# GabrielGao0310/SVT-av1_pro-anchor-v2.1.0-

Hardware: AMD Instinct MI355X
Metric: CDEF+restoration+SAD Mpixels/s on 4K10b (higher is better)
Workload: dtype u16

## Files before the change

svt-av1_pro-anchor-v2.1.0-_amd/csrc/dlf.hip:

```cpp
#include <algorithm>
#include <cstdlib>
#include <cstring>
#include <vector>

#include "svtgpu_internal.h"

#ifndef DLF_EXP
#define DLF_EXP 0
#endif

namespace {

constexpr int kNumBsize = 22;
__constant__ uint8_t c_tx_lw[3][kNumBsize] = {
    {2, 2, 3, 3, 3, 4, 4, 4, 5, 5, 5, 6, 6, 6, 6, 6, 2, 4, 3, 5, 4, 6},
    {2, 2, 3, 2, 3, 3, 3, 4, 4, 4, 5, 5, 5, 6, 6, 6, 2, 3, 3, 4, 4, 5},
    {2, 2, 3, 3, 2, 2, 2, 3, 3, 3, 4, 4, 4, 6, 6, 6, 2, 2, 3, 3, 4, 4}};
__constant__ uint8_t c_tx_lh[3][kNumBsize] = {
    {2, 3, 2, 3, 4, 3, 4, 5, 4, 5, 6, 5, 6, 6, 6, 6, 4, 2, 5, 3, 6, 4},
    {2, 3, 2, 2, 3, 3, 3, 4, 4, 4, 5, 5, 5, 6, 6, 6, 3, 2, 4, 3, 5, 4},
    {2, 3, 2, 3, 2, 2, 2, 3, 3, 3, 4, 4, 4, 6, 6, 6, 2, 2, 3, 3, 4, 4}};
__constant__ uint8_t c_uvtx_lw[kNumBsize] = {2, 2, 2, 2, 2, 3, 3, 3, 4, 4, 4, 5, 5, 5, 5, 5, 2, 3, 2, 4, 3, 5};
__constant__ uint8_t c_uvtx_lh[kNumBsize] = {2, 2, 2, 2, 3, 2, 3, 4, 3, 4, 5, 4, 5, 5, 5, 5, 3, 2, 4, 2, 5, 3};
__constant__ uint8_t c_bs_lw[kNumBsize]   = {2, 2, 3, 3, 3, 4, 4, 4, 5, 5, 5, 6, 6, 6, 7, 7, 2, 4, 3, 5, 4, 6};
__constant__ uint8_t c_bs_lh[kNumBsize]   = {2, 3, 2, 3, 4, 3, 4, 5, 4, 5, 6, 5, 6, 7, 6, 7, 4, 2, 5, 3, 6, 4};
__constant__ uint8_t c_uvbs_lw[kNumBsize] = {2, 2, 2, 2, 2, 3, 3, 3, 4, 4, 4, 5, 5, 5, 6, 6, 2, 3, 2, 4, 3, 5};
__constant__ uint8_t c_uvbs_lh[kNumBsize] = {2, 2, 2, 2, 3, 2, 3, 4, 3, 4, 5, 4, 5, 6, 5, 6, 3, 2, 4, 2, 5, 3};
__device__ __forceinline__ int mode_lf(int mode) { return mode >= 13 && mode != 15 && mode != 23; }

__device__ __forceinline__ int lf_class(const SvtGpuLfMi &m) {
    return m.segment_id * 16 + m.ref_frame0 * 2 + mode_lf(m.mode);
}

__device__ __forceinline__ int tx_log2(const SvtGpuLfMi &m, int vert, int chroma) {
    const int skipped = m.skip && m.ref_frame0 > 0;
    if (chroma) return vert ? c_uvtx_lw[m.bsize] : c_uvtx_lh[m.bsize];
    const int d = skipped ? 0 : m.tx_depth;
    return vert ? c_tx_lw[d][m.bsize] : c_tx_lh[d][m.bsize];
}

__device__ __forceinline__ SvtGpuLfMi checked_mi(SvtGpuLfMi m, unsigned long long *bad) {
    if (bad && (m.bsize >= kNumBsize || m.tx_depth > 2 || m.ref_frame0 < 0 || m.ref_frame0 > 7 || m.mode > 24 ||
                m.segment_id > 7)) {
        *bad = 1;
        m.bsize = min((int)m.bsize, kNumBsize - 1), m.tx_depth = min((int)m.tx_depth, 2);
        m.ref_frame0 = (int8_t)min(max((int)m.ref_frame0, 0), 7), m.mode = min((int)m.mode, 24);
        m.segment_id = min((int)m.segment_id, 7);
    }
    return m;
}

__global__ void dlf_edge_records_kernel(const SvtGpuLfMi *__restrict__ mi, int mi_cols, int units_w, int units_h,
                                        int chroma, int vert, int crop_w, int crop_h, uint32_t *__restrict__ rec,
                                        unsigned long long *bad) {
    const int ux = blockIdx.x * blockDim.x + threadIdx.x;
    const int uy = blockIdx.y;
    if (ux >= units_w || uy >= units_h) return;
    const int ss     = chroma;
    const int x      = ux * 4, y = uy * 4;
    const int mi_row = ss | ((y << ss) >> 2), mi_col = ss | ((x << ss) >> 2);
    const SvtGpuLfMi m = checked_mi(mi[mi_row * mi_cols + mi_col], bad);
    const int coord    = vert ? x : y;
    uint32_t  r        = 0;
    const int lt       = tx_log2(m, vert, chroma);
    if (coord && !(coord & ((1 << lt) - 1)) && x < crop_w && y < crop_h) {
        const SvtGpuLfMi p = checked_mi(vert ? mi[mi_row * mi_cols + mi_col - (1 << ss)]
                                             : mi[(mi_row - (1 << ss)) * mi_cols + mi_col], bad);
        const int cur_skip = m.skip && m.ref_frame0 > 0;
        const int pv_skip  = p.skip && p.ref_frame0 > 0;
        const int lpb      = chroma ? (vert ? c_uvbs_lw[m.bsize] : c_uvbs_lh[m.bsize])
                                    : (vert ? c_bs_lw[m.bsize] : c_bs_lh[m.bsize]);
        const int pu_edge  = !(coord & ((1 << lpb) - 1));
        if (!pv_skip || !cur_skip || pu_edge) {
            const int mlt = min(lt, tx_log2(p, vert, chroma));
            const int len = mlt == 2 ? 4 : chroma ? 6 : mlt == 3 ? 8 : 14;
            r = (uint32_t)len | ((uint32_t)lf_class(m) << 8) | ((uint32_t)lf_class(p) << 16);
        }
    }
    rec[(size_t)uy * units_w + ux] = r;
}

__device__ __forceinline__ int sclamp(int v, int lo, int hi) { return min(max(v, lo), hi); }

template <int N, int LOG2>
__device__ __forceinline__ void wide_filter(int *F) {
    int out[2 * N];
#pragma unroll
    for (int i = -N; i < N; i++) {
        int t = 0;
#pragma unroll
        for (int j = -N; j <= N; j++) {
            const int p   = min(max(i + j, -(N + 1)), N);
            const int tap = (N == 3 ? j == 0 : (j >= -1 && j <= 1)) ? 2 : 1;
            t += F[p + 7] * tap;
        }
        out[i + N] = (t + (1 << (LOG2 - 1))) >> LOG2;
    }
#pragma unroll
    for (int i = -N; i < N; i++) F[i + 7] = out[i + N];
}

__device__ __forceinline__ void filter_line(int *F, int len, int blimit, int limit, int thresh, int bd) {
    const int sh = bd - 8, one = 1 << sh;
    const int p3 = F[3], p2 = F[4], p1 = F[5], p0 = F[6], q0 = F[7], q1 = F[8], q2 = F[9], q3 = F[10];
    const int lim = limit << sh;
    if (abs(p0 - q0) * 2 + abs(p1 - q1) / 2 > (blimit << sh)) return;
    int m = max(abs(p1 - p0), abs(q1 - q0));
    int flat = 0;
    if (len >= 6) {
        m = max(m, max(abs(p2 - p1), abs(q2 - q1)));
        flat = max(max(abs(p1 - p0), abs(q1 - q0)), max(abs(p2 - p0), abs(q2 - q0)));
    }
    if (len >= 8) {
        m    = max(m, max(abs(p3 - p2), abs(q3 - q2)));
        flat = max(flat, max(abs(p3 - p0), abs(q3 - q0)));
    }
    if (m > lim) return;
    if (len >= 6 && flat <= one) {
        if (len == 14) {
            const int flat2 = max(max(max(abs(F[2] - p0), abs(F[11] - q0)), max(abs(F[1] - p0), abs(F[12] - q0))),
                                  max(abs(F[0] - p0), abs(F[13] - q0)));
            if (flat2 <= one) {
                wide_filter<6, 4>(F);
                return;
            }
        }
        if (len == 6)
            wide_filter<2, 3>(F);
        else
            wide_filter<3, 3>(F);
        return;
    }
    const int off = 0x80 << sh, lo = -(128 << sh), hi = (128 << sh) - 1;
    const bool hev = max(abs(p1 - p0), abs(q1 - q0)) > (thresh << sh);
    const int ps1 = p1 - off, ps0 = p0 - off, qs0 = q0 - off, qs1 = q1 - off;
    int f = hev ? sclamp(ps1 - qs1, lo, hi) : 0;
    f            = sclamp(f + 3 * (qs0 - ps0), lo, hi);
    const int f1 = sclamp(f + 4, lo, hi) >> 3;
    const int f2 = sclamp(f + 3, lo, hi) >> 3;
    F[7]         = sclamp(qs0 - f1, lo, hi) + off;
    F[6]         = sclamp(ps0 + f2, lo, hi) + off;
    if (!hev) {
        const int f3 = (f1 + 1) >> 1;
        F[8]         = sclamp(qs1 - f3, lo, hi) + off;
        F[5]         = sclamp(ps1 + f3, lo, hi) + off;
    }
}

__device__ __forceinline__ int half_taps(int len) { return len == 14 ? 7 : len == 8 ? 4 : len == 6 ? 3 : 2; }

constexpr int TILE  = 64;
constexpr int APRON = 12;
constexpr int LW    = TILE + 2 * APRON;
constexpr int NTHR  = 256;
constexpr int MAX_TRIALS = 2;

constexpr int MAX_JOBS   = 3;

struct DlfPlaneJob {
    int32_t         plane;
    const void     *src;
    void           *dst;
    const void     *ref;
    const uint32_t *rec_v, *rec_h;
    int32_t         src_stride, dst_stride, ref_stride;
    int32_t         units_w;
    int32_t         pw, ph, tiles_x, tiles;
    int32_t         ox, oy, ow, oh;
    int32_t         ntrial;
    uint8_t         lvl[MAX_TRIALS][2][128];
};

struct DlfDevPlan {
    int32_t ntrial[MAX_JOBS];
    int32_t lv[MAX_JOBS][MAX_TRIALS];
    uint8_t lvl[MAX_JOBS][MAX_TRIALS][2][128];
    int32_t done;
};

struct DlfTileArgs {
    DlfPlaneJob job[MAX_JOBS];
    int32_t     njob, bd;
    uint8_t     mblim[64], lim[64], hev[64];
    unsigned long long *sse;
    unsigned int       *arrive;
    unsigned long long *out;
    unsigned long long  seq;
    unsigned long long *wgclk;
    const DlfDevPlan   *plan;
    DlfDevPlan         *next_plan = nullptr;
    int32_t             dyn;
    const uint8_t      *dev_lvl;
};

typedef const __attribute__((address_space(4))) DlfTileArgs KArgs;
typedef const __attribute__((address_space(4))) DlfPlaneJob KJob;
__device__ __forceinline__ KArgs &kargs() { return *(KArgs *)__builtin_amdgcn_kernarg_segment_ptr(); }

struct DlfTileLds {
    uint16_t t[LW * LW];
    uint32_t rv[(LW / 4) * (TILE / 4 + 3)];
    uint32_t rh[(TILE / 4 + 3) * (TILE / 4)];
    unsigned long long red[NTHR / 64];
    uint8_t  s_lvl[2][128];
    uint32_t s_thr[64];
    uint16_t s_list[(LW / 4) * (TILE / 4 + 3)];
    int      s_cnt[8];
};

__device__ __forceinline__ int list_edges(const uint32_t *rec, int n, const uint8_t *lvl, uint16_t *list, int *s_cnt) {
    const int tid = threadIdx.x, lane = tid & 63;
    auto bucket = [&](int ri) {
        const uint32_t r   = rec[ri];
        const int      len = r & 15;
        if (!len || (!lvl[(r >> 8) & 127] && !lvl[(r >> 16) & 127])) return -1;
        return len == 4 ? 0 : len == 6 ? 1 : len == 8 ? 2 : 3;
    };
    if (tid < 8) s_cnt[tid] = 0;
    __syncthreads();
    for (int i0 = 0; i0 < n; i0 += NTHR) {
        const int b = i0 + tid < n ? bucket(i0 + tid) : -1;
#pragma unroll
        for (int g = 0; g < 4; g++) {
            const unsigned long long m = __ballot(b == g);
            if (m && lane == __ffsll((long long)m) - 1) atomicAdd(&s_cnt[g], (int)__popcll(m));
        }
    }
    __syncthreads();
    if (tid == 0) {
        int o = 0;
        for (int g = 0; g < 4; g++) {
            const int c = s_cnt[g];
            s_cnt[4 + g] = o, s_cnt[g] = o, o += c;
        }
    }
    __syncthreads();
    for (int i0 = 0; i0 < n; i0 += NTHR) {
        const int b = i0 + tid < n ? bucket(i0 + tid) : -1;
#pragma unroll
        for (int g = 0; g < 4; g++) {
            const unsigned long long m = __ballot(b == g);
            if (!m) continue;
            const int leader = __ffsll((long long)m) - 1;
            int       base   = 0;
            if (lane == leader) base = atomicAdd(&s_cnt[g], (int)__popcll(m));
            base = __shfl(base, leader);
            if (b == g) list[base + __popcll(m & ((1ull << lane) - 1))] = (uint16_t)(i0 + tid);
        }
    }
    __syncthreads();
    return s_cnt[3];
}

template <typename T, bool TRIAL>
__device__ __forceinline__ void dlf_tile_item(KArgs &a, int bi, int nbi, DlfTileLds &L) {
    uint16_t           *t = L.t;
    uint32_t           *rv = L.rv, *rh = L.rh;
    unsigned long long *red = L.red;
    uint8_t(*s_lvl)[128]   = L.s_lvl;
    uint32_t           *s_thr = L.s_thr;
    uint16_t           *s_list = L.s_list;
    int                *s_cnt = L.s_cnt;
    const int           tid = threadIdx.x;
    wgclk_mark(a.wgclk, 0);
    const int b = xcd_swizzle(bi, nbi);
#define DLF_NTR(j) (TRIAL ? (a.dyn ? a.plan->ntrial[j] : a.job[j].ntrial) : 1)
    int       jb = 0, tb = b;
    while (jb + 1 < a.njob && tb >= a.job[jb].tiles * DLF_NTR(jb)) tb -= a.job[jb].tiles * DLF_NTR(jb), jb++;
    KJob     &J  = a.job[jb];
    const int nt = DLF_NTR(jb);
#undef DLF_NTR
    if (TRIAL && nt == 0) return;
    const int tr = TRIAL ? tb % nt : 0;
    if (TRIAL) tb /= nt;
    if (TRIAL && a.plan && tr >= a.plan->ntrial[jb]) return;
    const int x0 = J.ox + (tb % J.tiles_x) * TILE, y0 = J.oy + (tb / J.tiles_x) * TILE;
    const int gx = x0 - APRON, gy = y0 - APRON;
    const T  *src = (const T *)J.src;
    __syncthreads();
    s_lvl[tid >> 7][tid & 127] = (TRIAL && a.plan) ? a.plan->lvl[jb][tr][tid >> 7][tid & 127]
                               : (!TRIAL && a.dev_lvl) ? a.dev_lvl[(J.plane * 2 + (tid >> 7)) * 128 + (tid & 127)]
                                                       : J.lvl[tr][tid >> 7][tid & 127];
    if (tid < 64) s_thr[tid] = (uint32_t)a.mblim[tid] | ((uint32_t)a.lim[tid] << 8) | ((uint32_t)a.hev[tid] << 16);

    constexpr int RV_R = LW / 4, RV_C = TILE / 4 + 3, RH_R = TILE / 4 + 3, RH_C = TILE / 4;
    constexpr int NV = RV_R * RV_C, NH = RH_R * RH_C, IR = (NV + NTHR - 1) / NTHR, IH = (NH + NTHR - 1) / NTHR;
    constexpr int NS = LW * LW / 4, IS = (NS + NTHR - 1) / NTHR;
    uint32_t      vrec[IR], hrec[IH];
    uint2         q[IS];
#pragma unroll
    for (int u = 0; u < IR; u++) {
        const int i = tid + u * NTHR, ur = gy / 4 + i / RV_C, uc = (x0 - 4) / 4 + i % RV_C;
        vrec[u] = (i < NV && ur >= 0 && uc >= 0 && ur * 4 < J.ph && uc * 4 < J.pw) ? J.rec_v[(size_t)ur * J.units_w + uc] : 0u;
    }
#pragma unroll
    for (int u = 0; u < IH; u++) {
        const int i = tid + u * NTHR, ur = (y0 - 4) / 4 + i / RH_C, uc = x0 / 4 + i % RH_C;
        hrec[u] = (i < NH && ur >= 0 && ur * 4 < J.ph && uc * 4 < J.pw) ? J.rec_h[(size_t)ur * J.units_w + uc] : 0u;
    }
#pragma unroll
    for (int u = 0; u < IS; u++) {
        const int i = tid + u * NTHR, r = gy + i / (LW / 4), c = gx + 4 * (i % (LW / 4));
        q[u] = make_uint2(0u, 0u);
        if (i >= NS || r < 0 || r >= J.ph) continue;
        const T *sp = src + (size_t)r * J.src_stride + c;
        if (c >= 0 && c + 4 <= J.pw) {
            if constexpr (sizeof(T) == 2) {
                q[u] = *(const uint2 *)sp;
            } else {
                const uint32_t b = *(const uint32_t *)sp;
                q[u] = make_uint2((b & 0xFF) | ((b & 0xFF00) << 8), ((b >> 16) & 0xFF) | ((b >> 8) & 0xFF0000));
            }
        } else {
            uint32_t w[2] = {0u, 0u};
#pragma unroll
            for (int j = 0; j < 4; j++)
                if (c + j >= 0 && c + j < J.pw) w[j >> 1] |= (uint32_t)(uint16_t)sp[j] << (16 * (j & 1));
            q[u] = make_uint2(w[0], w[1]);
        }
    }
#pragma unroll
    for (int u = 0; u < IR; u++)
        if (tid + u * NTHR < NV) rv[tid + u * NTHR] = vrec[u];
#pragma unroll
    for (int u = 0; u < IH; u++)
        if (tid + u * NTHR < NH) rh[tid + u * NTHR] = hrec[u];
#pragma unroll
    for (int u = 0; u < IS; u++)
        if (tid + u * NTHR < NS) *(uint2 *)&t[4 * (tid + u * NTHR)] = q[u];
    const int tw = min(TILE, J.ox + J.ow - x0), th = min(TILE, J.oy + J.oh - y0);
    {
        __syncthreads();
        wgclk_mark(a.wgclk, 1);
        const int nve = list_edges(rv, NV, s_lvl[0], s_list, s_cnt);
        for (int i = tid; i < ((DLF_EXP & 1) ? 0 : nve * 4); i += NTHR) {
            const int ri = s_list[i >> 2], line = i & 3, e = ri % RV_C, sr = ri / RV_C;
            const uint32_t r = rv[ri];
            const int len = r & 15;
            const int cur = s_lvl[0][(r >> 8) & 127], prv = s_lvl[0][(r >> 16) & 127];
            const uint32_t th = s_thr[cur ? cur : prv];
            uint16_t *row = &t[(sr * 4 + line) * LW + (APRON - 4 + e * 4)];
            const int h = half_taps(len);
            int F[14];
#pragma unroll
            for (int k = 0; k < 14; k++) F[k] = (k >= 7 - h && k < 7 + h) ? row[k - 7] : 0;
            filter_line(F, len, th & 0xFF, (th >> 8) & 0xFF, th >> 16, a.bd);
#pragma unroll
            for (int k = 0; k < 14; k++)
                if (k >= 7 - h && k < 7 + h) row[k - 7] = (uint16_t)F[k];
        }
        __syncthreads();
        wgclk_mark(a.wgclk, 2);
        const int nhe = list_edges(rh, NH, s_lvl[1], s_list, s_cnt);
        for (int i = tid; i < ((DLF_EXP & 2) ? 0 : nhe * 4); i += NTHR) {
            const int ri = s_list[i >> 2], e = ri / RH_C, col = 4 * (ri % RH_C) + (i & 3);
            const uint32_t r = rh[ri];
            const int len = r & 15;
            const int cur = s_lvl[1][(r >> 8) & 127], prv = s_lvl[1][(r >> 16) & 127];
            const uint32_t th = s_thr[cur ? cur : prv];
            uint16_t *c = &t[(APRON - 4 + e * 4) * LW + APRON + col];
            const int h = half_taps(len);
            int F[14];
#pragma unroll
            for (int k = 0; k < 14; k++) F[k] = (k >= 7 - h && k < 7 + h) ? c[(k - 7) * LW] : 0;
            filter_line(F, len, th & 0xFF, (th >> 8) & 0xFF, th >> 16, a.bd);
#pragma unroll
            for (int k = 0; k < 14; k++)
                if (k >= 7 - h && k < 7 + h) c[(k - 7) * LW] = (uint16_t)F[k];
        }
        __syncthreads();
        wgclk_mark(a.wgclk, 3);
        if (TRIAL) {
            uint32_t  s = 0;
            const T  *ref = (const T *)J.ref;
            const int c = tid % TILE;
            if (c < tw) {
                int rv16[TILE / (NTHR / TILE)];
#pragma unroll
                for (int k = 0; k < TILE / (NTHR / TILE); k++) {
                    const int r = tid / TILE + k * (NTHR / TILE);
                    rv16[k] = r < th ? (int)ref[(size_t)(y0 + r) * J.ref_stride + x0 + c] : 0;
                }
#pragma unroll
                for (int k = 0; k < TILE / (NTHR / TILE); k++) {
                    const int r = tid / TILE + k * (NTHR / TILE);
                    const int d = r < th ? (int)t[(APRON + r) * LW + APRON + c] - rv16[k] : 0;
                    s += (uint32_t)(d * d);
                }
            }
            const unsigned long long sw = wave_sum_u32_wide(s);
            if ((tid & 63) == 63) red[tid >> 6] = sw;
            __syncthreads();
            if (tid == 0) {
                unsigned long long tot = 0;
                for (int w = 0; w < NTHR / 64; w++) tot += red[w];
                atomicAdd(&a.sse[jb * MAX_TRIALS + tr], tot);
            }
        } else {
            T *dst = (T *)J.dst;
            for (int i = tid; i < TILE * TILE / 4; i += NTHR) {
                const int r = i / (TILE / 4), c = 4 * (i % (TILE / 4));
                if (r >= th || c >= tw) continue;
                const uint2 w = *(const uint2 *)&t[(APRON + r) * LW + APRON + c];
                T *d = dst + (size_t)(y0 + r) * J.dst_stride + x0 + c;
                if constexpr (sizeof(T) == 2)
                    *(uint2 *)d = w;
                else
                    *(uint32_t *)d = (w.x & 0xFF) | ((w.x >> 8) & 0xFF00) | ((w.y & 0xFF) << 16) | ((w.y & 0xFF0000) << 8);
            }
        }
    }
    wgclk_mark(a.wgclk, 5);
}

template <typename T, bool TRIAL>
__global__ __launch_bounds__(NTHR, 8) void dlf_tile_kernel(const DlfTileArgs a0) {
    __shared__ __align__(16) DlfTileLds L;
    KArgs    &a   = kargs();
    const int tid = threadIdx.x;
    dlf_tile_item<T, TRIAL>(a, blockIdx.x, gridDim.x, L);
    if (TRIAL && tid == 0 && !a.plan) {
        asm volatile("s_waitcnt vmcnt(0)" ::: "memory");
        if (atomicAdd(a.arrive, 1u) == gridDim.x - 1) {
            for (int q = 0; q < MAX_JOBS * MAX_TRIALS; q++) a.out[q] = atomicExch(&a.sse[q], 0ull);
            atomicExch(a.arrive, 0u);
            __threadfence_system();
            __hip_atomic_store(&a.out[MAX_JOBS * MAX_TRIALS], a.seq, __ATOMIC_RELAXED, __HIP_MEMORY_SCOPE_SYSTEM);
        }
    }
}

template <typename T>
__global__ __launch_bounds__(256) void plane_sse_kernel(const T *a, int as, const T *b, int bs, int w, int h,
                                                        unsigned long long *out) {
    __shared__ unsigned long long red[4];
    unsigned long long s = 0;
    for (int r = blockIdx.x; r < h; r += gridDim.x)
        for (int c = threadIdx.x; c < w; c += 256) {
            const int d = (int)a[(size_t)r * as + c] - (int)b[(size_t)r * bs + c];
            s += (unsigned long long)(d * d);
        }
    s = wave_sum_lane63(s);
    if ((threadIdx.x & 63) == 63) red[threadIdx.x >> 6] = s;
    __syncthreads();
    if (threadIdx.x == 0) atomicAdd(out, red[0] + red[1] + red[2] + red[3]);
}

__global__ void lpf_lines_kernel(uint16_t *lines, int len, int blimit, int limit, int thresh, int bd) {
    const int l = threadIdx.x;
    if (l >= 4) return;
    int F[14];
    for (int k = 0; k < 14; k++) F[k] = lines[l * 16 + 1 + k];
    filter_line(F, len, blimit, limit, thresh, bd);
    for (int k = 0; k < 14; k++) lines[l * 16 + 1 + k] = (uint16_t)F[k];
}

}

struct SvtGpuDlfState {
    SvtGpuContext *ctx;
    int32_t        width, height, mi_rows, mi_cols;
    SvtGpuLfMi    *d_mi;
    uint32_t      *d_rec[2][2];
    int32_t        uw[2], uh[2];
    int32_t        crop_w, crop_h;
    void          *d_scratch;
    unsigned long long *d_sse;
    unsigned int       *d_arrive;
    unsigned long long *h_sse;
    unsigned long long *h_sse_dev;
    unsigned long long  seq;
    int32_t        have_mi;
    int32_t        mi_on_device = 0;
    int32_t        sse_rect[4] = {0, 0, 0, 0}, out_rect[4] = {0, 0, 0, 0};
    SvtGpuComm    *comm = nullptr;
    void          *d_search = nullptr;
    void          *d_plans  = nullptr;
    void          *h_search = nullptr;
    SvtGpuLfMi    *h_mi = nullptr;
    SvtGpuPrioLane prio;
    hipEvent_t     mi_free = nullptr;
    void          *d_res = nullptr, *h_res = nullptr, *h_res_dev = nullptr;
    int32_t        dev_seq = 0, dev_pending = 0, dev_ready = 0, dev_rounds = 8, dev_rounds_last = 0, dev_seen = 0;
    SvtGpuLfParams dev_params{};
};

namespace {

struct LevelTables {
    uint8_t lvl[3][2][128];
    uint8_t mblim[64], lim[64], hev[64];
};

__host__ __device__ static inline int clampi(int v, int lo, int hi) { return v < lo ? lo : v > hi ? hi : v; }

__host__ __device__ static inline uint8_t level_entry(const SvtGpuLfParams &p, int pl, int dir, int lv, int cls) {
    const int feat[3][2] = {{1, 2}, {3, 3}, {4, 4}};
    const int seg = cls >> 4, ref = (cls >> 1) & 7, mode = cls & 1;
    int       ls  = lv;
    if (p.segmentation_enabled && p.seg_feature_enabled[seg][feat[pl][dir]])
        ls = clampi(ls + p.seg_feature_data[seg][feat[pl][dir]], 0, 63);
    int v = ls;
    if (p.mode_ref_delta_enabled) {
        const int scale = 1 << (ls >> 5);
        v = ls + p.ref_deltas[ref] * scale + (ref > 0 ? p.mode_deltas[mode] * scale : 0);
        v = clampi(v, 0, 63);
    }
    return (uint8_t)v;
}

__host__ __device__ static void fill_level_table(const SvtGpuLfParams &p, int pl, int dir, int lv, uint8_t *out) {
    for (int cls = 0; cls < 128; cls++) out[cls] = level_entry(p, pl, dir, lv, cls);
}

void build_level_tables(const SvtGpuLfParams &p, LevelTables &L) {
    std::memset(&L, 0, sizeof L);
    const int sh = p.sharpness_level;
    for (int l = 0; l < 64; l++) {
        int inside = l >> ((sh > 0) + (sh > 4));
        if (sh > 0) inside = std::min(inside, 9 - sh);
        inside     = std::max(inside, 1);
        L.lim[l]   = (uint8_t)inside;
        L.mblim[l] = (uint8_t)(2 * (l + 2) + inside);
        L.hev[l]   = (uint8_t)(l >> 4);
    }
    const int base[3][2] = {{p.filter_level[0], p.filter_level[1]},
                            {p.filter_level_u, p.filter_level_u},
                            {p.filter_level_v, p.filter_level_v}};
    for (int pl = 0; pl < 3; pl++)
        for (int dir = 0; dir < 2; dir++) fill_level_table(p, pl, dir, base[pl][dir], L.lvl[pl][dir]);
}

__host__ __device__ bool plane_active(const SvtGpuLfParams &p, int plane) {
    if (plane == 0) return p.filter_level[0] || p.filter_level[1];
    return plane == 1 ? p.filter_level_u != 0 : p.filter_level_v != 0;
}

DlfPlaneJob plane_job(SvtGpuDlfState *s, const SvtGpuFrame *f, int plane, bool trial) {
    DlfPlaneJob j;
    std::memset(&j, 0, sizeof j);
    j.plane   = plane;
    const int ch = plane > 0;
    j.rec_v   = s->d_rec[ch][0];
    j.rec_h   = s->d_rec[ch][1];
    j.units_w = s->uw[ch];
    j.pw      = f->pw[plane];
    j.ph      = f->ph[plane];
    const int32_t *r = trial ? s->sse_rect : s->out_rect;
    const int      sh = plane > 0;
    j.ox      = r[0] >> sh, j.oy = r[1] >> sh;
    j.ow      = std::min(j.pw, (r[2] + sh) >> sh) - j.ox, j.oh = std::min(j.ph, (r[3] + sh) >> sh) - j.oy;
    j.tiles_x = (j.ow + TILE - 1) / TILE;
    j.tiles   = j.ow > 0 && j.oh > 0 ? j.tiles_x * ((j.oh + TILE - 1) / TILE) : 0;
    return j;
}

DlfTileArgs base_args(const SvtGpuFrame *f, const LevelTables &L) {
    DlfTileArgs a;
    std::memset(&a, 0, sizeof a);
    a.bd = f->bit_depth;
    std::memcpy(a.mblim, L.mblim, 64);
    std::memcpy(a.lim, L.lim, 64);
    std::memcpy(a.hev, L.hev, 64);
    return a;
}

int launch_tile(const DlfTileArgs &a0, int bps, bool trial, hipStream_t st) {
    int tiles = 0;
    for (int j = 0; j < a0.njob; j++) tiles += a0.job[j].tiles * (trial ? a0.job[j].ntrial : 1);
    DlfTileArgs a = a0;
    a.wgclk       = svtgpu_wgclk_begin(tiles);
    if (bps == 2) {
        if (trial) hipLaunchKernelGGL((dlf_tile_kernel<uint16_t, true>), dim3(tiles), dim3(NTHR), 0, st, a);
        else       hipLaunchKernelGGL((dlf_tile_kernel<uint16_t, false>), dim3(tiles), dim3(NTHR), 0, st, a);
    } else {
        if (trial) hipLaunchKernelGGL((dlf_tile_kernel<uint8_t, true>), dim3(tiles), dim3(NTHR), 0, st, a);
        else       hipLaunchKernelGGL((dlf_tile_kernel<uint8_t, false>), dim3(tiles), dim3(NTHR), 0, st, a);
    }
    HIP_TRY(hipGetLastError());
    svtgpu_wgclk_end(trial ? "dlf_trial" : "dlf_apply", tiles, st);
    return SVTGPU_OK;
}

bool frame_matches(const SvtGpuDlfState *s, const SvtGpuFrame *f) {
    return f && f->width == s->width && f->height == s->height && (f->bit_depth == 8 || f->bit_depth == 10);
}

__host__ __device__ void set_trial_level(SvtGpuLfParams &p, int plane, int dir, int lvl) {
    if (plane == 0) {
        if (dir != 1) p.filter_level[0] = lvl;
        if (dir != 0) p.filter_level[1] = lvl;
    } else if (plane == 1)
        p.filter_level_u = lvl;
    else
        p.filter_level_v = lvl;
}

struct LevelSearch {
    int     plane = 0, dir = 0, early_exit = 0, only4x4 = 0;
    int     mid = 0, step = 0, direction = 0, conv = 0, best = 0;
    int64_t best_err = 0, bias = 0, err[64];
    int     phase = 0;
    int     lo = 0, hi = 0;
    bool    try_lo = false, try_hi = false;
    int     req[MAX_TRIALS], nreq = 0;

    __host__ __device__ LevelSearch() {}
    __host__ __device__ LevelSearch(const int last[4], int dlf_avg, int early_exit_, int only4x4_, int plane_, int dir_)
        : plane(plane_), dir(dir_), early_exit(early_exit_), only4x4(only4x4_) {
        const int start = plane == 0 ? (dlf_avg ? last[0] : last[dir]) : last[plane + 1];
        mid  = clampi(start, 0, 63);
        step = mid < 16 ? 4 : mid / 4;
        best = mid;
        for (int i = 0; i < 64; i++) err[i] = -1;
        req[0] = mid, nreq = 1;
    }
    __host__ __device__ void next_request() {
        if (step <= 0) {
            phase = 2, nreq = 0;
            return;
        }
        hi   = mid + step < 63 ? mid + step : 63, lo = mid - step > 0 ? mid - step : 0;
        bias = (best_err >> (15 - (mid / 8))) * step;
        if (!only4x4) bias >>= 1;
        try_lo = direction <= 0 && lo != mid, try_hi = direction >= 0 && hi != mid;
        nreq   = 0;
        if (try_lo) req[nreq++] = lo;
        if (try_hi) req[nreq++] = hi;
    }
    __host__ __device__ void resolve() {
        if (phase == 0) {
            best_err = err[mid], best = mid, phase = 1;
        } else {
            if (try_lo && err[lo] < best_err + bias) {
                if (err[lo] < best_err) best_err = err[lo];
                best = lo;
            }
            if (try_hi && err[hi] < best_err - bias) {
                best_err = err[hi];
                best     = hi;
            }
            if (best == mid) {
                conv++;
                step      = conv == early_exit ? 0 : step / 2;
                direction = 0;
            } else {
                direction = best < mid ? -1 : 1;
                mid       = best;
            }
        }
        next_request();
    }
    __host__ __device__ int pending(int *lv) {
        while (phase != 2) {
            int m = 0;
            for (int k = 0; k < nreq; k++) {
                bool dup = err[req[k]] >= 0;
                for (int j = 0; j < m && !dup; j++) dup = lv[j] == req[k];
                if (!dup) lv[m++] = req[k];
            }
            if (m) return m;
            resolve();
        }
        return 0;
    }
    __host__ __device__ void feed(const int *lv, int m, const unsigned long long *sse) {
        for (int k = 0; k < m; k++) err[lv[k]] = (int64_t)sse[k];
    }
};

struct DlfDevSearch {
    LevelSearch    srch[MAX_JOBS];
    int32_t        ns;
    SvtGpuLfParams p;
    DlfDevPlan     plan;
    int32_t        rounds;
};
struct DlfDevResult {
    int32_t levels[4];
    int32_t rounds, seq, pad[2];
    uint8_t lvl[3][2][128];
};

__host__ __device__ void plan_levels(DlfDevSearch &S) {
    S.plan.done = 1;
    for (int i = 0; i < MAX_JOBS; i++) {
        const int m = i < S.ns ? S.srch[i].pending(S.plan.lv[i]) : 0;
        S.plan.ntrial[i] = m;
        if (m) S.plan.done = 0;
    }
}
// ... 714 lines not shown
```

Baseline: 3286.

## Prune apron deblock edges, vectorize LDS filter I/O, prefetch trial reference

Adds a per-column row-range analysis from the horizontal-edge lengths so that vertical edges in apron rows that cannot affect the output tile are skipped. Boundary horizontal edges are dropped unless they use 14-tap filters. The vertical-edge filter now reads and writes LDS pixels with packed 32/64-bit accesses instead of per-pixel ones. The trial-mode reference pixels are loaded into registers before the filter passes to hide global latency. The edge-bucketing loop is templated so bucket results are cached in registers rather than recomputed. The pruning relies on tap-reach reasoning, and a mistake there would give incorrect pixels at tile borders.

```diff
diff --git a/svt-av1_pro-anchor-v2.1.0-_amd/csrc/dlf.hip b/svt-av1_pro-anchor-v2.1.0-_amd/csrc/dlf.hip
--- a/svt-av1_pro-anchor-v2.1.0-_amd/csrc/dlf.hip
+++ b/svt-av1_pro-anchor-v2.1.0-_amd/csrc/dlf.hip
@@ -206,20 +206,34 @@
     uint32_t s_thr[64];
     uint16_t s_list[(LW / 4) * (TILE / 4 + 3)];
     int      s_cnt[8];
+    uint8_t  s_unit[2][TILE / 4];
 };
 
-__device__ __forceinline__ int list_edges(const uint32_t *rec, int n, const uint8_t *lvl, uint16_t *list, int *s_cnt) {
+__device__ __forceinline__ bool need_vert_unit(const uint8_t (*unit)[TILE / 4], int e, int sr, int len) {
+    const int c0 = max(e - (len == 14 ? 3 : 2), 0), c1 = min(len == 14 ? e : e - 1, TILE / 4 - 1);
+    int lo = 255, hi = -1;
+#pragma unroll
+    for (int k = 0; k < 4; k++)
+        if (c0 + k <= c1) lo = min(lo, (int)unit[0][c0 + k]), hi = max(hi, (int)unit[1][c0 + k]);
+    return sr >= lo && sr <= hi;
+}
+
+template <int N, typename Keep>
+__device__ __forceinline__ int list_edges(const uint32_t *rec, const uint8_t *lvl, uint16_t *list, int *s_cnt, Keep keep) {
+    constexpr int IT = (N + NTHR - 1) / NTHR;
     const int tid = threadIdx.x, lane = tid & 63;
     auto bucket = [&](int ri) {
         const uint32_t r   = rec[ri];
         const int      len = r & 15;
-        if (!len || (!lvl[(r >> 8) & 127] && !lvl[(r >> 16) & 127])) return -1;
+        if (!len || (!lvl[(r >> 8) & 127] && !lvl[(r >> 16) & 127]) || !keep(ri, len)) return -1;
         return len == 4 ? 0 : len == 6 ? 1 : len == 8 ? 2 : 3;
     };
+    int bk[IT];
     if (tid < 8) s_cnt[tid] = 0;
     __syncthreads();
-    for (int i0 = 0; i0 < n; i0 += NTHR) {
-        const int b = i0 + tid < n ? bucket(i0 + tid) : -1;
+#pragma unroll
+    for (int u = 0; u < IT; u++) {
+        const int b = bk[u] = u * NTHR + tid < N ? bucket(u * NTHR + tid) : -1;
 #pragma unroll
         for (int g = 0; g < 4; g++) {
             const unsigned long long m = __ballot(b == g);
@@ -235,8 +249,9 @@
         }
     }
     __syncthreads();
-    for (int i0 = 0; i0 < n; i0 += NTHR) {
-        const int b = i0 + tid < n ? bucket(i0 + tid) : -1;
+#pragma unroll
+    for (int u = 0; u < IT; u++) {
+        const int b = bk[u];
 #pragma unroll
         for (int g = 0; g < 4; g++) {
             const unsigned long long m = __ballot(b == g);
@@ -245,7 +260,7 @@
             int       base   = 0;
             if (lane == leader) base = atomicAdd(&s_cnt[g], (int)__popcll(m));
             base = __shfl(base, leader);
-            if (b == g) list[base + __popcll(m & ((1ull << lane) - 1))] = (uint16_t)(i0 + tid);
+            if (b == g) list[base + __popcll(m & ((1ull << lane) - 1))] = (uint16_t)(u * NTHR + tid);
         }
     }
     __syncthreads();
@@ -329,10 +344,45 @@
     for (int u = 0; u < IS; u++)
         if (tid + u * NTHR < NS) *(uint2 *)&t[4 * (tid + u * NTHR)] = q[u];
     const int tw = min(TILE, J.ox + J.ow - x0), th = min(TILE, J.oy + J.oh - y0);
+    constexpr int ER = TILE * TILE / 4 / NTHR, EC = TILE / 4;
+    uint2         ref4[TRIAL ? ER : 1];
+    if (TRIAL) {
+        const T  *ref = (const T *)J.ref;
+        const int c = 4 * (tid % EC);
+#pragma unroll
+        for (int k = 0; k < ER; k++) {
+            const int r = tid / EC + k * (NTHR / EC);
+            ref4[k] = make_uint2(0u, 0u);
+            if (r >= th || c >= tw) continue;
+            const T *sp = ref + (size_t)(y0 + r) * J.ref_stride + x0 + c;
+            if (c + 4 <= tw) {
+                if constexpr (sizeof(T) == 2) {
+                    ref4[k] = *(const uint2 *)sp;
+                } else {
+                    const uint32_t b = *(const uint32_t *)sp;
+                    ref4[k] = make_uint2((b & 0xFF) | ((b & 0xFF00) << 8), ((b >> 16) & 0xFF) | ((b >> 8) & 0xFF0000));
+                }
+            } else {
+                uint32_t w[2] = {0u, 0u};
+#pragma unroll
+                for (int j = 0; j < 4; j++)
+                    if (c + j < tw) w[j >> 1] |= (uint32_t)(uint16_t)sp[j] << (16 * (j & 1));
+                ref4[k] = make_uint2(w[0], w[1]);
+            }
+        }
+    }
     {
         __syncthreads();
         wgclk_mark(a.wgclk, 1);
-        const int nve = list_edges(rv, NV, s_lvl[0], s_list, s_cnt);
+        if (tid < TILE / 4) {
+            const int l0 = rh[tid] & 15, l1 = rh[RH_C + tid] & 15;
+            const int l17 = rh[17 * RH_C + tid] & 15, l18 = rh[18 * RH_C + tid] & 15;
+            L.s_unit[0][tid] = (uint8_t)(l0 == 14 ? 0 : l1 == 14 ? 1 : l1 ? 2 : 3);
+            L.s_unit[1][tid] = (uint8_t)(l18 == 14 ? 21 : l17 == 14 ? 20 : l17 ? 19 : 18);
+        }
+        const int nve = list_edges<NV>(rv, s_lvl[0], s_list, s_cnt, [&](int ri, int len) {
+            return need_vert_unit(L.s_unit, ri % RV_C, ri / RV_C, len);
+        });
         for (int i = tid; i < ((DLF_EXP & 1) ? 0 : nve * 4); i += NTHR) {
             const int ri = s_list[i >> 2], line = i & 3, e = ri % RV_C, sr = ri / RV_C;
             const uint32_t r = rv[ri];
@@ -340,18 +390,31 @@
             const int cur = s_lvl[0][(r >> 8) & 127], prv = s_lvl[0][(r >> 16) & 127];
             const uint32_t th = s_thr[cur ? cur : prv];
             uint16_t *row = &t[(sr * 4 + line) * LW + (APRON - 4 + e * 4)];
-            const int h = half_taps(len);
-            int F[14];
-#pragma unroll
-            for (int k = 0; k < 14; k++) F[k] = (k >= 7 - h && k < 7 + h) ? row[k - 7] : 0;
+            const uint2 m0 = *(const uint2 *)(row - 4), m1 = *(const uint2 *)row;
+            uint2       o0 = make_uint2(0u, 0u), o1 = o0;
+            if (len == 14) o0 = *(const uint2 *)(row - 8), o1 = *(const uint2 *)(row + 4);
+            int F[14] = {(int)(o0.x >> 16), (int)(o0.y & 0xFFFF), (int)(o0.y >> 16), (int)(m0.x & 0xFFFF),
+                         (int)(m0.x >> 16), (int)(m0.y & 0xFFFF), (int)(m0.y >> 16), (int)(m1.x & 0xFFFF),
+                         (int)(m1.x >> 16), (int)(m1.y & 0xFFFF), (int)(m1.y >> 16), (int)(o1.x & 0xFFFF),
+                         (int)(o1.x >> 16), (int)(o1.y & 0xFFFF)};
             filter_line(F, len, th & 0xFF, (th >> 8) & 0xFF, th >> 16, a.bd);
-#pragma unroll
-            for (int k = 0; k < 14; k++)
-                if (k >= 7 - h && k < 7 + h) row[k - 7] = (uint16_t)F[k];
+            const uint32_t w1 = (uint32_t)F[5] | ((uint32_t)F[6] << 16), w2 = (uint32_t)F[7] | ((uint32_t)F[8] << 16);
+            if (len < 8) {
+                *(uint32_t *)(row - 2) = w1, *(uint32_t *)row = w2;
+            } else {
+                *(uint2 *)(row - 4) = make_uint2((uint32_t)F[3] | ((uint32_t)F[4] << 16), w1);
+                *(uint2 *)row       = make_uint2(w2, (uint32_t)F[9] | ((uint32_t)F[10] << 16));
+                if (len == 14) {
+                    *(uint32_t *)(row - 6) = (uint32_t)F[1] | ((uint32_t)F[2] << 16);
+                    *(uint32_t *)(row + 4) = (uint32_t)F[11] | ((uint32_t)F[12] << 16);
+                }
+            }
         }
         __syncthreads();
         wgclk_mark(a.wgclk, 2);
-        const int nhe = list_edges(rh, NH, s_lvl[1], s_list, s_cnt);
+        const int nhe = list_edges<NH>(rh, s_lvl[1], s_list, s_cnt, [&](int ri, int len) {
+            return (ri >= RH_C && ri < (RH_R - 1) * RH_C) || len == 14;
+        });
         for (int i = tid; i < ((DLF_EXP & 2) ? 0 : nhe * 4); i += NTHR) {
             const int ri = s_list[i >> 2], e = ri / RH_C, col = 4 * (ri % RH_C) + (i & 3);
             const uint32_t r = rh[ri];
@@ -372,21 +435,17 @@
         wgclk_mark(a.wgclk, 3);
         if (TRIAL) {
             uint32_t  s = 0;
-            const T  *ref = (const T *)J.ref;
-            const int c = tid % TILE;
-            if (c < tw) {
-                int rv16[TILE / (NTHR / TILE)];
-#pragma unroll
-                for (int k = 0; k < TILE / (NTHR / TILE); k++) {
-                    const int r = tid / TILE + k * (NTHR / TILE);
-                    rv16[k] = r < th ? (int)ref[(size_t)(y0 + r) * J.ref_stride + x0 + c] : 0;
-                }
-#pragma unroll
-                for (int k = 0; k < TILE / (NTHR / TILE); k++) {
-                    const int r = tid / TILE + k * (NTHR / TILE);
-                    const int d = r < th ? (int)t[(APRON + r) * LW + APRON + c] - rv16[k] : 0;
-                    s += (uint32_t)(d * d);
-                }
+            const int c = 4 * (tid % EC);
+#pragma unroll
+            for (int k = 0; k < ER; k++) {
+                const int r = tid / EC + k * (NTHR / EC);
+                if (r >= th) continue;
+                const uint2 w = *(const uint2 *)&t[(APRON + r) * LW + APRON + c];
+                const int   d[4] = {(int)(w.x & 0xFFFF) - (int)(ref4[k].x & 0xFFFF), (int)(w.x >> 16) - (int)(ref4[k].x >> 16),
+                                    (int)(w.y & 0xFFFF) - (int)(ref4[k].y & 0xFFFF), (int)(w.y >> 16) - (int)(ref4[k].y >> 16)};
+#pragma unroll
+                for (int j = 0; j < 4; j++)
+                    if (c + j < tw) s += (uint32_t)(d[j] * d[j]);
             }
             const unsigned long long sw = wave_sum_u32_wide(s);
             if ((tid & 63) == 63) red[tid >> 6] = sw;
```

After: 3370 (median of 6 runs). +2.6%, better.
